# pythoncrazy/jimm

Measured on NVIDIA H100. Metric: images/sec, higher is better.
Workload: dtype f16

## Files before the change

jimm_b200/csrc/common.cuh:

```cuda
#pragma once

#include <cuda.h>
#include <cuda_bf16.h>
#include <cuda_fp16.h>
#include <cuda_fp8.h>
#include <cuda_runtime.h>
#include <stdint.h>

#include <atomic>
#include <mutex>
#include <string>

namespace jimm {

void set_last_error(const char* fmt, ...);

#define JIMM_CUDA_CHECK(expr)                                                                   \
  do {                                                                                          \
    cudaError_t _e = (expr);                                                                    \
    if (_e != cudaSuccess) {                                                                    \
      ::jimm::set_last_error("%s:%d: %s -> %s", __FILE__, __LINE__, #expr, cudaGetErrorString(_e)); \
      return -2;                                                                                \
    }                                                                                           \
  } while (0)
// ... 80 lines not shown
      : "=r"(pred));
  return pred != 0;
}

__device__ __forceinline__ void mbar_init(uint64_t* bar, uint32_t count) {
  asm volatile("mbarrier.init.shared::cta.b64 [%0], %1;" ::"r"(smem_u32(bar)), "r"(count));
}
__device__ __forceinline__ void fence_barrier_init() {
  asm volatile("fence.mbarrier_init.release.cluster;" ::: "memory");
}
__device__ __forceinline__ void fence_proxy_async_smem() {
  asm volatile("fence.proxy.async.shared::cta;" ::: "memory");
}
__device__ __forceinline__ void mbar_arrive(uint64_t* bar) {
  asm volatile("mbarrier.arrive.shared::cta.b64 _, [%0];" ::"r"(smem_u32(bar)) : "memory");
}
__device__ __forceinline__ void mbar_arrive_expect_tx(uint64_t* bar, uint32_t bytes) {
  asm volatile("mbarrier.arrive.expect_tx.shared::cta.b64 _, [%0], %1;" ::"r"(smem_u32(bar)), "r"(bytes) : "memory");
}
__device__ __forceinline__ void mbar_wait(uint64_t* bar, uint32_t parity) {
  asm volatile(
      "{\n\t.reg .pred P1;\n\t"
      "WAIT_LOOP:\n\t"
      "mbarrier.try_wait.parity.shared::cta.b64 P1, [%0], %1;\n\t"
      "@P1 bra DONE;\n\t"
      "bra WAIT_LOOP;\n\t"
      "DONE:\n\t}" ::"r"(smem_u32(bar)),
      "r"(parity)
      : "memory");
}

__device__ __forceinline__ bool mbar_test_wait(uint64_t* bar, uint32_t parity) {
  uint32_t ok;
  asm volatile(
      "{\n\t.reg .pred P1;\n\t"
      "mbarrier.test_wait.parity.shared::cta.b64 P1, [%1], %2;\n\t"
      "selp.u32 %0, 1, 0, P1;\n\t}"
      : "=r"(ok)
      : "r"(smem_u32(bar)), "r"(parity)
      : "memory");
  return ok != 0;
}

__device__ __forceinline__ void tma_prefetch_desc(const CUtensorMap* m) {
  asm volatile("prefetch.tensormap [%0];" ::"l"(reinterpret_cast<uint64_t>(m)) : "memory");
}
__device__ __forceinline__ void tma_load_2d(void* smem_dst, const CUtensorMap* m, uint64_t* bar, int c0, int c1) {
  asm volatile(
      "cp.async.bulk.tensor.2d.shared::cluster.global.mbarrier::complete_tx::bytes [%0], [%1, {%3, %4}], [%2];" ::"r"(
          smem_u32(smem_dst)),
      "l"(reinterpret_cast<uint64_t>(m)), "r"(smem_u32(bar)), "r"(c0), "r"(c1)
      : "memory");
}

__device__ __forceinline__ void tma_store_2d(const CUtensorMap* m, uint32_t smem_src, int c0, int c1) {
  asm volatile("cp.async.bulk.tensor.2d.global.shared::cta.bulk_group [%0, {%2, %3}], [%1];" ::"l"(reinterpret_cast<uint64_t>(m)),
               "r"(smem_src), "r"(c0), "r"(c1)
               : "memory");
}
__device__ __forceinline__ void tma_reduce_add_2d(const CUtensorMap* m, uint32_t smem_src, int c0, int c1) {
  asm volatile("cp.reduce.async.bulk.tensor.2d.global.shared::cta.add.tile.bulk_group [%0, {%2, %3}], [%1];" ::"l"(
                   reinterpret_cast<uint64_t>(m)),
               "r"(smem_src), "r"(c0), "r"(c1)
               : "memory");
}
__device__ __forceinline__ void tma_store_3d(const CUtensorMap* m, uint32_t smem_src, int c0, int c1, int c2) {
  asm volatile("cp.async.bulk.tensor.3d.global.shared::cta.bulk_group [%0, {%2, %3, %4}], [%1];" ::"l"(reinterpret_cast<uint64_t>(m)),
               "r"(smem_src), "r"(c0), "r"(c1), "r"(c2)
               : "memory");
}
__device__ __forceinline__ void tma_reduce_add_3d(const CUtensorMap* m, uint32_t smem_src, int c0, int c1, int c2) {
  asm volatile("cp.reduce.async.bulk.tensor.3d.global.shared::cta.add.tile.bulk_group [%0, {%2, %3, %4}], [%1];" ::"l"(
                   reinterpret_cast<uint64_t>(m)),
               "r"(smem_src), "r"(c0), "r"(c1), "r"(c2)
               : "memory");
}
__device__ __forceinline__ void tma_store_commit() { asm volatile("cp.async.bulk.commit_group;" ::: "memory"); }
__device__ __forceinline__ void tma_store_wait_read() { asm volatile("cp.async.bulk.wait_group.read 0;" ::: "memory"); }
__device__ __forceinline__ void tma_store_wait_read1() { asm volatile("cp.async.bulk.wait_group.read 1;" ::: "memory"); }
__device__ __forceinline__ void tma_store_wait_all() { asm volatile("cp.async.bulk.wait_group 0;" ::: "memory"); }

__device__ __forceinline__ uint32_t cluster_ctarank() {
  uint32_t r;
  asm volatile("mov.u32 %0, %%cluster_ctarank;" : "=r"(r));
  return r;
}
__device__ __forceinline__ void cluster_sync_all() {
  asm volatile("barrier.cluster.arrive.release.aligned;\n\tbarrier.cluster.wait.acquire.aligned;" ::: "memory");
}
__device__ __forceinline__ uint32_t mapa_shared(uint32_t local_smem_addr, uint32_t rank) {
  uint32_t r;
  asm volatile("mapa.shared::cluster.u32 %0, %1, %2;" : "=r"(r) : "r"(local_smem_addr), "r"(rank));
  return r;
}
__device__ __forceinline__ void mbar_arrive_cluster(uint32_t cluster_addr) {
  asm volatile("mbarrier.arrive.release.cluster.shared::cluster.b64 _, [%0];" ::"r"(cluster_addr) : "memory");
}
__device__ __forceinline__ uint64_t make_wgmma_desc_sw128(uint32_t smem_addr) {
  uint64_t d = 0;
  d |= static_cast<uint64_t>((smem_addr & 0x3FFFFu) >> 4);
  d |= static_cast<uint64_t>(1) << 16;
  d |= static_cast<uint64_t>(1024 >> 4) << 32;
  d |= static_cast<uint64_t>(1) << 62;
  return d;
}
template <int SW>
__device__ __forceinline__ uint64_t make_wgmma_desc(uint32_t smem_addr, uint32_t lbo) {
  static_assert(SW == 128 || SW == 64 || SW == 32, "swizzle width");
  constexpr uint64_t layout = SW == 128 ? 1 : SW == 64 ? 2 : 3;
  uint64_t d = 0;
  d |= static_cast<uint64_t>((smem_addr & 0x3FFFFu) >> 4);
  d |= static_cast<uint64_t>((lbo >> 4) & 0x3FFFu) << 16;
  d |= static_cast<uint64_t>(8 * SW >> 4) << 32;
  d |= layout << 62;
  return d;
}
__device__ __forceinline__ void wgmma_fence() { asm volatile("wgmma.fence.sync.aligned;" ::: "memory"); }
__device__ __forceinline__ void wgmma_commit() { asm volatile("wgmma.commit_group.sync.aligned;" ::: "memory"); }
template <int N>
__device__ __forceinline__ void wgmma_wait() { asm volatile("wgmma.wait_group.sync.aligned %0;" ::"n"(N) : "memory"); }
template <int R>
__device__ __forceinline__ void wgmma_fence_operands(float (&d)[R]) {
#pragma unroll
  for (int i = 0; i < R; ++i) asm volatile("" : "+f"(d[i])::"memory");
}

#define JIMM_WGMMA_D128                                                                                                                    \
  "{%0, %1, %2, %3, %4, %5, %6, %7, %8, %9, %10, %11, %12, %13, %14, %15, %16, %17, %18, %19, %20, %21, %22, %23, %24, %25, %26, %27, "     \
  "%28, %29, %30, %31, %32, %33, %34, %35, %36, %37, %38, %39, %40, %41, %42, %43, %44, %45, %46, %47, %48, %49, %50, %51, %52, %53, %54, " \
  "%55, %56, %57, %58, %59, %60, %61, %62, %63, %64, %65, %66, %67, %68, %69, %70, %71, %72, %73, %74, %75, %76, %77, %78, %79, %80, %81, " \
  "%82, %83, %84, %85, %86, %87, %88, %89, %90, %91, %92, %93, %94, %95, %96, %97, %98, %99, %100, %101, %102, %103, %104, %105, %106, "   \
  "%107, %108, %109, %110, %111, %112, %113, %114, %115, %116, %117, %118, %119, %120, %121, %122, %123, %124, %125, %126, %127}"
#define JIMM_WGMMA_D8(i) "+f"(d[i]), "+f"(d[i + 1]), "+f"(d[i + 2]), "+f"(d[i + 3]), "+f"(d[i + 4]), "+f"(d[i + 5]), "+f"(d[i + 6]), "+f"(d[i + 7])
#define JIMM_WGMMA_D128_OPERANDS                                                                                                 \
  JIMM_WGMMA_D8(0), JIMM_WGMMA_D8(8), JIMM_WGMMA_D8(16), JIMM_WGMMA_D8(24), JIMM_WGMMA_D8(32), JIMM_WGMMA_D8(40), JIMM_WGMMA_D8(48), \
      JIMM_WGMMA_D8(56), JIMM_WGMMA_D8(64), JIMM_WGMMA_D8(72), JIMM_WGMMA_D8(80), JIMM_WGMMA_D8(88), JIMM_WGMMA_D8(96),             \
      JIMM_WGMMA_D8(104), JIMM_WGMMA_D8(112), JIMM_WGMMA_D8(120)
template <int KIND>
__device__ __forceinline__ void wgmma_m64n256_ss(float (&d)[128], uint64_t adesc, uint64_t bdesc, uint32_t accumulate) {
  if constexpr (KIND == 0) {
    asm volatile("{\n\t.reg .pred p;\n\tsetp.ne.b32 p, %130, 0;\n\t"
                 "wgmma.mma_async.sync.aligned.m64n256k16.f32.f16.f16 " JIMM_WGMMA_D128 ", %128, %129, p, 1, 1, 0, 0;\n\t}"
                 : JIMM_WGMMA_D128_OPERANDS
                 : "l"(adesc), "l"(bdesc), "r"(accumulate));
  } else if constexpr (KIND == 1) {
    asm volatile("{\n\t.reg .pred p;\n\tsetp.ne.b32 p, %130, 0;\n\t"
                 "wgmma.mma_async.sync.aligned.m64n256k16.f32.bf16.bf16 " JIMM_WGMMA_D128 ", %128, %129, p, 1, 1, 0, 0;\n\t}"
                 : JIMM_WGMMA_D128_OPERANDS
                 : "l"(adesc), "l"(bdesc), "r"(accumulate));
// ... 260 lines not shown
```

jimm_b200/csrc/gemm.cu:

```cuda
#include "gemm.cuh"

#include <stdarg.h>
#include <stdio.h>
#include <stdlib.h>
#include <string.h>

#include <type_traits>

#include "common.cuh"

namespace jimm {

static constexpr int BM = GEMM_TILE_M;
static constexpr int BN = GEMM_TILE_N;
static_assert(BM == 128 && BN == 256, "the warp roles and the wgmma shape below are written for 128 x 256 tiles");
static constexpr int STAGES = 4;
static constexpr int A_STAGE_BYTES = BM * 128;
static constexpr int B_STAGE_BYTES = BN * 128;
static constexpr int STAGE_BYTES = A_STAGE_BYTES + B_STAGE_BYTES;
static constexpr int EPI_WARPS = 8;
static constexpr int EPI_BOX_ROWS = 16;
static constexpr int EPI_BUF_BYTES = EPI_BOX_ROWS * 128;
static constexpr int EPI_BUFS = 2;
static constexpr int EPI_STAGE_BYTES = EPI_WARPS * EPI_BUFS * EPI_BUF_BYTES;
static constexpr int NUM_THREADS = 384;
static constexpr int KERNEL_REGS = 168;

enum OutKind : int { OUT_GENERIC = 0, OUT_H16 = 1, OUT_BF16 = 2, OUT_TF32 = 3, OUT_F32_ADD = 4, OUT_F32 = 5 };

struct EpiDev {
  const float* bias;
  const float* rowadd;
  const float* residual;
  void* out;
  int act, ldr, out_type, ldo, rows_in, rows_out, row_off, mode;
  int M, N;
  int reverse;
  int tok_pad, tok_off;
  const float* ln_scale;
  const float* ln_bias;
  void* ln_out;
  int* ln_cnt;
  int ln_out_type, ln_ldo;
  float ln_eps;
  const float* a_scale;
  const float* b_scale;
};

template <int ACT>
__device__ __forceinline__ float act_ct(float v) {
  if constexpr (ACT == ACT_GELU_TANH) return gelu_tanh(v);
  else if constexpr (ACT == ACT_QUICK_GELU) return quick_gelu(v);
  else return v;
}
__device__ __forceinline__ float apply_act(float v, int act) {
  if (act == ACT_GELU_TANH) return gelu_tanh(v);
  if (act == ACT_QUICK_GELU) return quick_gelu(v);
  return v;
}

__device__ __forceinline__ void remap_row(const EpiDev& e, int row, int& out_row, int& add_row) {
  if (e.rows_in > 0) {
    int b = row / e.rows_in, p = row - b * e.rows_in;
    out_row = b * e.rows_out + p + e.row_off;
    add_row = p + e.row_off;
  } else {
    out_row = row;
    add_row = row;
  }
}

// ... 239 lines not shown
    int out_row, add_row;
    remap_row(epi, row, out_row, add_row);
    float sa = 1.f;
    if constexpr (SCALED) sa = __ldg(epi.a_scale + row);
#pragma unroll
    for (int j = 0; j < NC / 8; ++j) {
#pragma unroll
      for (int q = 0; q < 2; ++q) {
        const int col = n_tile0 + 8 * j + 2 * t + q;
        if (col < epi.N) {
          float v = acc[4 * j + 2 * h + q];
          if constexpr (SCALED) v *= sa * __ldg(epi.b_scale + col);
          if (epi.bias) v += __ldg(epi.bias + col);
          v = apply_act(v, epi.act);
          if (epi.rowadd) v += __ldg(epi.rowadd + static_cast<size_t>(add_row) * epi.N + col);
          if (epi.residual) v += epi.residual[static_cast<size_t>(out_row) * epi.ldr + col];
          store1(epi, out_row, col, v);
        }
      }
    }
  }
}


template <typename T, int OUT, int ACT>
__global__ void __launch_bounds__(NUM_THREADS, 1)
gemm_wgmma_kernel(const __grid_constant__ CUtensorMap map_a, const __grid_constant__ CUtensorMap map_b,
                  const __grid_constant__ CUtensorMap map_c, const EpiDev epi, int K) {
  constexpr bool SCALED = kScaled<T>;
  constexpr int BK = 128 / sizeof(T);
  constexpr int UK = 32 / sizeof(T);
  constexpr int TM = tile_rows(Traits<T>::DTYPE);
  constexpr int STAGE_TX = TM * 128 + B_STAGE_BYTES;
  constexpr int WG_DM = SCALED ? 0 : 64;
  constexpr int WG_DN = SCALED ? 128 : 0;
  constexpr int NC = BN - WG_DN;
  constexpr bool FUSE_LN = OUT == OUT_F32_ADD && ACT == ACT_FUSE_LN;
  constexpr int EPI_ACT = ACT == ACT_FUSE_LN ? static_cast<int>(ACT_NONE) : ACT;
  constexpr int PRODUCER_REGS = FUSE_LN ? 152 : 40;
  constexpr int CONSUMER_REGS = FUSE_LN ? 176 : 232;
  static_assert(128 * PRODUCER_REGS + 256 * CONSUMER_REGS <= NUM_THREADS * KERNEL_REGS, "register split exceeds the CTA's allocation");

  extern __shared__ uint8_t smem_raw[];
  uint8_t* smem = reinterpret_cast<uint8_t*>((reinterpret_cast<uintptr_t>(smem_raw) + 1023) & ~static_cast<uintptr_t>(1023));
  uint8_t* smem_a = smem;
  uint8_t* smem_b = smem + STAGES * A_STAGE_BYTES;
  uint8_t* epi_stage = smem + STAGES * STAGE_BYTES;
  LnQueue* lnq = reinterpret_cast<LnQueue*>(epi_stage + EPI_STAGE_BYTES);
  uint64_t* full_bar = reinterpret_cast<uint64_t*>(lnq + 1);
  uint64_t* empty_bar = full_bar + STAGES;

  const int warp_idx = threadIdx.x >> 5;
  const int lane = threadIdx.x & 31;
  const int M = epi.M, N = epi.N;
  const int m_tiles = (M + TM - 1) / TM, n_tiles = (N + BN - 1) / BN;
  const int num_tiles = m_tiles * n_tiles;
  const int num_kb = (K + BK - 1) / BK;

  pdl_launch_dependents();
  if (warp_idx == 0 && lane == 0) {
    tma_prefetch_desc(&map_a);
    tma_prefetch_desc(&map_b);
    if constexpr (OUT != OUT_GENERIC) tma_prefetch_desc(&map_c);
    for (int s = 0; s < STAGES; ++s) {
      mbar_init(&full_bar[s], 1);
      mbar_init(&empty_bar[s], EPI_WARPS);
    }
    fence_barrier_init();
  }
  if constexpr (FUSE_LN) {
    if (warp_idx == 1) {
      for (int i = lane; i < LNQ; i += 32) lnq->slot[i] = -1;
      if (lane == 0) lnq->head = lnq->tail = lnq->done = 0;
    }
  }
  __syncthreads();
  pdl_wait();

  if (warp_idx < 4) {
    setmaxnreg<KERNEL_REGS, PRODUCER_REGS>();
    if (warp_idx == 0) {
      if (lane == 0) {
        int stage = 0;
        uint32_t phase = 0;
        for (int tile = blockIdx.x; tile < num_tiles; tile += gridDim.x) {
          const int tv = epi.reverse ? num_tiles - 1 - tile : tile;
          const int m_blk = tv / n_tiles, n_blk = tv - m_blk * n_tiles;
          for (int kb = 0; kb < num_kb; ++kb) {
            mbar_wait(&empty_bar[stage], phase ^ 1);
            mbar_arrive_expect_tx(&full_bar[stage], STAGE_TX);
            tma_load_2d(smem_a + stage * A_STAGE_BYTES, &map_a, &full_bar[stage], kb * BK, m_blk * TM);
            tma_load_2d(smem_b + stage * B_STAGE_BYTES, &map_b, &full_bar[stage], kb * BK, n_blk * BN);
            if (++stage == STAGES) { stage = 0; phase ^= 1; }
          }
        }
      }
    } else if constexpr (FUSE_LN) {
      ln_worker<T>(epi, lnq, lane);
    }
  } else {
    setmaxnreg<KERNEL_REGS, CONSUMER_REGS>();
    const int wg = (warp_idx - 4) >> 2;
    const int wq = warp_idx & 3;
    uint8_t* tbuf0 = epi_stage + (warp_idx - 4) * EPI_BUFS * EPI_BUF_BYTES;
    int stage = 0;
    uint32_t phase = 0, box_count = 0;
    int ln_rg = -1, ln_cols = 0;
    float acc[NC / 2];
    for (int tile = blockIdx.x; tile < num_tiles; tile += gridDim.x) {
      const int tv = epi.reverse ? num_tiles - 1 - tile : tile;
      const int m_blk = tv / n_tiles, n_blk = tv - m_blk * n_tiles;
      int prev = -1;
      if constexpr (SCALED) {
#pragma unroll
        for (int i = 0; i < NC / 2; ++i) acc[i] = 0.f;
      }
      for (int kb = 0; kb < num_kb; ++kb) {
        mbar_wait(&full_bar[stage], phase);
        const uint64_t adesc = make_wgmma_desc_sw128(smem_u32(smem_a + stage * A_STAGE_BYTES + wg * WG_DM * 128));
        const uint64_t bdesc = make_wgmma_desc_sw128(smem_u32(smem_b + stage * B_STAGE_BYTES + wg * WG_DN * 128));
        if constexpr (SCALED) {
          float slab[NC / 2];
          wgmma_fence_operands(slab);
          wgmma_fence();
#pragma unroll
          for (int k = 0; k < BK / UK; ++k)
            wgmma_m64n128k32_e4m3_ss(slab, adesc + static_cast<uint64_t>(2 * k), bdesc + static_cast<uint64_t>(2 * k), k != 0 ? 1u : 0u);
          wgmma_commit();
          wgmma_wait<0>();
          wgmma_fence_operands(slab);
          if (lane == 0) mbar_arrive(&empty_bar[stage]);
#pragma unroll
          for (int i = 0; i < NC / 2; ++i) acc[i] += slab[i];
        } else {
          wgmma_fence_operands(acc);
          wgmma_fence();
#pragma unroll
          for (int k = 0; k < BK / UK; ++k)
            wgmma_m64n256_ss<Traits<T>::KIND>(acc, adesc + static_cast<uint64_t>(2 * k), bdesc + static_cast<uint64_t>(2 * k), (kb | k) != 0 ? 1u : 0u);
          wgmma_commit();
          wgmma_fence_operands(acc);
          if (prev >= 0) {
            wgmma_wait<1>();
            if (lane == 0) mbar_arrive(&empty_bar[prev]);
          }
          prev = stage;
        }
        if (++stage == STAGES) { stage = 0; phase ^= 1; }
      }
      if constexpr (!SCALED) {
        wgmma_wait<0>();
        wgmma_fence_operands(acc);
        if (lane == 0) mbar_arrive(&empty_bar[prev]);
      }

      const int row_base = m_blk * TM + wg * WG_DM + wq * 16;
      const int n_tile0 = n_blk * BN + wg * WG_DN;
      if constexpr (OUT == OUT_GENERIC) {
        epilogue_generic<SCALED, NC>(epi, acc, lane, row_base, n_tile0);
      } else {
        if (row_base < M && (WG_DN == 0 || n_tile0 < N))
          epilogue_tma<OUT, EPI_ACT, SCALED, NC>(&map_c, epi, acc, tbuf0, lane, row_base, n_tile0, box_count);
        if constexpr (FUSE_LN) {
          if (lane == 0 && ln_rg >= 0) ln_publish(epi, lnq, ln_rg, ln_cols);
          ln_rg = (row_base & ~31) < M ? row_base >> 5 : -1;
          ln_cols = min(BN, N - n_tile0);
        }
      }
    }
    if constexpr (FUSE_LN) {
      if (lane == 0) {
        if (ln_rg >= 0) ln_publish(epi, lnq, ln_rg, ln_cols);
        __threadfence_block();
        atomicAdd(&lnq->done, 1);
      }
    }
    if constexpr (OUT != OUT_GENERIC) {
      if (lane == 0) tma_store_wait_all();
    }
  }
}

template <typename T>
__global__ void gemm_simt_kernel(const T* __restrict__ A, int lda, const T* __restrict__ B, int ldb, int K, EpiDev epi) {
  __shared__ float As[16][17], Bs[16][17];
  const int tx = threadIdx.x, ty = threadIdx.y;
  const int row = blockIdx.y * 16 + ty, col = blockIdx.x * 16 + tx;
  float acc = 0.f;
  for (int k0 = 0; k0 < K; k0 += 16) {
    const int ar = blockIdx.y * 16 + ty, ak = k0 + tx;
    As[ty][tx] = (ar < epi.M && ak < K) ? to_float(A[static_cast<size_t>(ar) * lda + ak]) : 0.f;
    const int br = blockIdx.x * 16 + ty, bk = k0 + tx;
    Bs[ty][tx] = (br < epi.N && bk < K) ? to_float(B[static_cast<size_t>(br) * ldb + bk]) : 0.f;
    __syncthreads();
#pragma unroll
    for (int k = 0; k < 16; ++k) acc += As[ty][k] * Bs[tx][k];
    __syncthreads();
  }
  if (row < epi.M && col < epi.N) {
    int out_row, add_row;
    remap_row(epi, row, out_row, add_row);
    float v = acc;
    if constexpr (kScaled<T>) v *= epi.a_scale[row] * epi.b_scale[col];
    if (epi.bias) v += epi.bias[col];
    v = apply_act(v, epi.act);
    if (epi.rowadd) v += epi.rowadd[static_cast<size_t>(add_row) * epi.N + col];
    if (epi.residual) v += epi.residual[static_cast<size_t>(out_row) * epi.ldr + col];
    store1(epi, out_row, col, v);
  }
}

static constexpr int SMEM_BYTES = STAGES * STAGE_BYTES + EPI_STAGE_BYTES + static_cast<int>(sizeof(LnQueue)) + 2 * STAGES * 8 + 1024;
static_assert(SMEM_BYTES <= 232448, "exceeds 227 KB of shared memory");
typedef CUresult (*PFN_encodeTiled)(CUtensorMap*, CUtensorMapDataType, cuuint32_t, void*, const cuuint64_t*, const cuuint64_t*,
                                    const cuuint32_t*, const cuuint32_t*, CUtensorMapInterleave, CUtensorMapSwizzle,
                                    CUtensorMapL2promotion, CUtensorMapFloatOOBfill);

static PFN_encodeTiled get_encode_fn() {
  static std::atomic<PFN_encodeTiled> fn{nullptr};
  if (PFN_encodeTiled f = fn.load(std::memory_order_acquire)) return f;
  void* p = nullptr;
  cudaDriverEntryPointQueryResult qres;
  cudaError_t e = cudaGetDriverEntryPoint("cuTensorMapEncodeTiled", &p, cudaEnableDefault, &qres);
  if (e != cudaSuccess || qres != cudaDriverEntryPointSuccess || p == nullptr) {
    set_last_error("cudaGetDriverEntryPoint(cuTensorMapEncodeTiled) failed: %s", cudaGetErrorString(e));
    return nullptr;
  }
  fn.store(reinterpret_cast<PFN_encodeTiled>(p), std::memory_order_release);
  return reinterpret_cast<PFN_encodeTiled>(p);
}

static CUtensorMapDataType tensor_map_dtype(int dtype) {
  switch (dtype) {
// ... 39 lines not shown
  if (r != CUDA_SUCCESS) { set_last_error("cuTensorMapEncodeTiled(3d) failed: CUresult %d", static_cast<int>(r)); return -3; }
  return 0;
}

int device_sm_count() {
  static std::atomic<int> sms[DeviceOnce::kMaxDevices] = {};
  int dev = 0;
  cudaGetDevice(&dev);
  if (dev < 0 || dev >= DeviceOnce::kMaxDevices) dev = 0;
  int n = sms[dev].load(std::memory_order_relaxed);
  if (n == 0) {
    cudaDeviceGetAttribute(&n, cudaDevAttrMultiProcessorCount, dev);
    const char* env = getenv("JIMM_NUM_SMS");
    if (env && atoi(env) > 0) n = atoi(env);
    sms[dev].store(n, std::memory_order_relaxed);
  }
  return n;
}

static int check_epi(const GemmEpilogue& e, int N) {
  if (e.out == nullptr) { set_last_error("gemm: null output"); return -1; }
  if (e.ldo < N) { set_last_error("gemm: ldo (%d) < N (%d)", e.ldo, N); return -1; }
  return 0;
}
static int check_e4m3_epi(const GemmEpilogue& e) {
  if (e.a_scale == nullptr || e.b_scale == nullptr) { set_last_error("gemm: e4m3 operands need row scales for A and B"); return -1; }
  if ((reinterpret_cast<uintptr_t>(e.b_scale) & 7) != 0) { set_last_error("gemm: the B scales must be 8-byte aligned"); return -1; }
  if (e.residual || e.rowadd || e.rows_in != 0 || e.tok_pad != 0 || e.ln_cnt) {
    set_last_error("gemm: e4m3 operands support bias and activation epilogues only (no residual, row-add, row remap, token scatter or "
                   "fused LayerNorm)");
    return -1;
  }
  return 0;
}
int gemm_plan_init(GemmPlan* plan, int dtype, const void* A, int lda, const void* B, int ldb, int M, int N, int K,
                   const GemmEpilogue& epi) {
  if (M <= 0 || N <= 0 || K <= 0) { set_last_error("gemm: bad shape %dx%dx%d", M, N, K); return -1; }
  if (int rc = check_epi(epi, N)) return rc;
  if (dtype == DT_E4M3) {
    if (int rc = check_e4m3_epi(epi)) return rc;
  }
  if (epi.tok_pad != 0) {
    if (epi.tok_pad < 0 || epi.tok_pad % EPI_BOX_ROWS != 0 || M % epi.tok_pad != 0 || epi.tok_off < 0 || epi.tok_S <= 0) {
      set_last_error("gemm: token scatter needs tok_pad a positive multiple of %d dividing M (tok_pad=%d M=%d tok_off=%d tok_S=%d)", EPI_BOX_ROWS,
                     epi.tok_pad, M, epi.tok_off, epi.tok_S);
      return -1;
    }
    if (epi.residual != epi.out || epi.ldr != epi.ldo || epi.out_type != DT_F32) {
      set_last_error("gemm: token scatter reduce-adds into an fp32 output that is also the residual");
      return -1;
    }
  }
  if (int rc = make_tensor_map_2d(&plan->map_a, dtype, A, M, K, lda, tile_rows(dtype))) return rc;
  if (int rc = make_tensor_map_2d(&plan->map_b, dtype, B, N, K, ldb, BN)) return rc;
  plan->M = M; plan->N = N; plan->K = K; plan->dtype = dtype; plan->epi = epi;
  memset(&plan->map_c, 0, sizeof(plan->map_c));
  if (plan->epi.mode == 2) {
    const size_t es = dtype_size(epi.out_type);
    const bool ok = epi.rowadd == nullptr && epi.rows_in == 0 && (static_cast<size_t>(N) * es) % 16 == 0 &&
                    (epi.residual == nullptr || (epi.residual == epi.out && epi.ldr == epi.ldo && epi.out_type == DT_F32)) &&
                    (static_cast<size_t>(epi.ldo) * es) % 16 == 0 && (reinterpret_cast<uintptr_t>(epi.out) & 15) == 0 &&
                    (epi.bias == nullptr || ((reinterpret_cast<uintptr_t>(epi.bias) & 15) == 0 && N % 4 == 0)) &&
                    !(epi.residual && epi.act != ACT_NONE);
    if (ok && epi.tok_pad > 0) {
      if (int rc = make_tensor_map_3d(&plan->map_c, DT_F32, epi.out, M / epi.tok_pad, epi.tok_S, N, epi.ldo)) return rc;
    } else if (ok) {
      if (int rc = make_tensor_map_2d(&plan->map_c, epi.out_type, epi.out, M, N, epi.ldo, EPI_BOX_ROWS)) return rc;
    } else {
      plan->epi.mode = 0;
    }
  }
  if (epi.tok_pad > 0 && plan->epi.mode != 2) {
    set_last_error("gemm: the token scatter needs the TMA epilogue (mode 2, no activation, 16-byte aligned output / bias, N %% 4 == 0)");
    return -1;
  }
  return 0;
}

static EpiDev to_dev(const GemmEpilogue& e, int M, int N) {
  EpiDev d;
  d.bias = e.bias; d.rowadd = e.rowadd; d.residual = e.residual; d.out = e.out;
  d.act = e.act; d.ldr = e.ldr; d.out_type = e.out_type; d.ldo = e.ldo;
  d.rows_in = e.rows_in; d.rows_out = e.rows_out; d.row_off = e.row_off; d.mode = e.mode;
  d.M = M; d.N = N;
  d.tok_pad = e.tok_pad; d.tok_off = e.tok_off;
  d.reverse = e.reverse;
  d.ln_scale = e.ln_scale; d.ln_bias = e.ln_bias; d.ln_out = e.ln_out; d.ln_cnt = e.ln_cnt;
  d.ln_out_type = e.ln_out_type; d.ln_ldo = e.ln_ldo; d.ln_eps = e.ln_eps;
  d.a_scale = e.a_scale; d.b_scale = e.b_scale;
  return d;
}

template <typename T, int OUT, int ACT>
static int launch_one(const GemmPlan* p, int M, cudaStream_t stream) {
  auto* kernel = gemm_wgmma_kernel<T, OUT, ACT>;
  constexpr int TM = tile_rows(Traits<T>::DTYPE);
  static DeviceOnce attr_set;
  if (int rc = attr_set.run([&]() -> int {
        JIMM_CUDA_CHECK(cudaFuncSetAttribute(kernel, cudaFuncAttributeMaxDynamicSharedMemorySize, SMEM_BYTES));
        cudaFuncAttributes fa;
        JIMM_CUDA_CHECK(cudaFuncGetAttributes(&fa, kernel));
        if (fa.numRegs != KERNEL_REGS) {
          set_last_error("gemm: kernel compiled with %d registers per thread, the warpgroup register split assumes %d", fa.numRegs, KERNEL_REGS);
          return -2;
        }
        return 0;
      }))
    return rc;
  const int tiles = ((M + TM - 1) / TM) * ((p->N + BN - 1) / BN);
  const int grid = tiles < device_sm_count() ? tiles : device_sm_count();
  JIMM_CUDA_CHECK(launch_k(kernel, dim3(grid), dim3(NUM_THREADS), SMEM_BYTES, stream, 1, true, p->map_a, p->map_b, p->map_c,
                           to_dev(p->epi, M, p->N), p->K));
  note_launch();
  return 0;
}

template <typename T, int OUT>
static int launch_act(const GemmPlan* p, int M, cudaStream_t stream) {
  switch (p->epi.act) {
    case ACT_GELU_TANH: return launch_one<T, OUT, ACT_GELU_TANH>(p, M, stream);
    case ACT_QUICK_GELU: return launch_one<T, OUT, ACT_QUICK_GELU>(p, M, stream);
    default: return launch_one<T, OUT, ACT_NONE>(p, M, stream);
  }
}

template <typename T>
static int launch_tc(const GemmPlan* p, int M, cudaStream_t stream) {
  const GemmEpilogue& e = p->epi;
  if (e.mode != 2) return launch_one<T, OUT_GENERIC, ACT_NONE>(p, M, stream);
  if constexpr (!kScaled<T>) {
    if (e.residual) return gemm_fuses_ln(p, M) ? launch_one<T, OUT_F32_ADD, ACT_FUSE_LN>(p, M, stream) : launch_one<T, OUT_F32_ADD, ACT_NONE>(p, M, stream);
  }
  switch (e.out_type) {
    case DT_F16: return launch_act<T, OUT_H16>(p, M, stream);
    case DT_BF16: return launch_act<T, OUT_BF16>(p, M, stream);
    case DT_TF32: return launch_act<T, OUT_TF32>(p, M, stream);
    default: return launch_act<T, OUT_F32>(p, M, stream);
  }
}

int gemm_fuses_ln(const GemmPlan* p, int ) {
  const int nv = p->N >> 7;
  const bool width_ok = p->N % 128 == 0 && (nv <= 4 || nv == 6 || nv == 8 || nv == 9);
  const int want = p->dtype == DT_F16 ? DT_F16 : p->dtype == DT_BF16 ? DT_BF16 : DT_TF32;
  return p->epi.ln_cnt != nullptr && p->epi.ln_out_type == want && width_ok && p->epi.mode == 2 && p->epi.residual != nullptr && p->epi.tok_pad == 0;
}

int gemm_plan_run(const GemmPlan* p0, int M_override, cudaStream_t stream, int reverse) {
  const int M = (M_override > 0 && M_override <= p0->M) ? M_override : p0->M;
  if (p0->epi.tok_pad > 0 && M % p0->epi.tok_pad != 0) {
    set_last_error("gemm: token scatter runs whole samples (M=%d, tok_pad=%d)", M, p0->epi.tok_pad);
    return -1;
  }
  GemmPlan local;
  const GemmPlan* p = p0;
  if (reverse != p0->epi.reverse) { local = *p0; local.epi.reverse = reverse; p = &local; }
  switch (p->dtype) {
    case DT_F16: return launch_tc<__half>(p, M, stream);
    case DT_BF16: return launch_tc<__nv_bfloat16>(p, M, stream);
    case DT_F32:
    case DT_TF32: return launch_tc<float>(p, M, stream);
    case DT_E4M3: return launch_tc<__nv_fp8_e4m3>(p, M, stream);
  }
  set_last_error("gemm: bad dtype %d", p->dtype);
// ... 21 lines not shown
```

jimm_b200/csrc/gemm.cuh:

```cuda
#pragma once
#include <cuda.h>
#include <cuda_runtime.h>
#include <stdint.h>

namespace jimm {

enum DType : int { DT_F32 = 0, DT_F16 = 1, DT_BF16 = 2, DT_TF32 = 3, DT_E4M3 = 4 };
enum Act : int { ACT_NONE = 0, ACT_GELU_TANH = 1, ACT_QUICK_GELU = 2 };

inline size_t dtype_size(int dt) { return (dt == DT_F32 || dt == DT_TF32) ? 4 : dt == DT_E4M3 ? 1 : 2; }

constexpr int GEMM_TILE_M = 128;
constexpr int GEMM_TILE_N = 256;

struct GemmEpilogue {
  const float* bias = nullptr;
  int act = ACT_NONE;
  const float* rowadd = nullptr;
  const float* residual = nullptr;
  int ldr = 0;
  void* out = nullptr;
  int out_type = DT_F32;
  int ldo = 0;
  int tok_pad = 0, tok_off = 0, tok_S = 0;
  int reverse = 0;
  int rows_in = 0, rows_out = 0, row_off = 0;
  int mode = 2;
  const float* ln_scale = nullptr;
  const float* ln_bias = nullptr;
  void* ln_out = nullptr;
  int ln_out_type = DT_F16, ln_ldo = 0;
  float ln_eps = 1e-6f;
  int* ln_cnt = nullptr;
  const float* a_scale = nullptr;
  const float* b_scale = nullptr;
};

struct GemmPlan {
  CUtensorMap map_a, map_b, map_c;
  int M = 0, N = 0, K = 0;
  int dtype = DT_F16;
  GemmEpilogue epi;
};

int gemm_plan_init(GemmPlan* plan, int dtype, const void* A, int lda, const void* B, int ldb, int M, int N, int K,
                   const GemmEpilogue& epi);
int gemm_plan_run(const GemmPlan* plan, int M_override, cudaStream_t stream, int reverse = 0);

int gemm_simt_run(int dtype, const void* A, int lda, const void* B, int ldb, int M, int N, int K, const GemmEpilogue& epi,
                  cudaStream_t stream);

int gemm_fuses_ln(const GemmPlan* plan, int M_override);

int device_sm_count();

}
```

jimm_b200/csrc/model.cu:

```cuda
#include <stdarg.h>
#include <stdio.h>
#include <stdlib.h>
#include <string.h>

#include <algorithm>
#include <atomic>
#include <cmath>
#include <map>
#include <tuple>
#include <memory>
#include <utility>
#include <string>
#include <vector>

#include "../../include/jimm_b200.h"
#include "comm.cuh"
#include "common.cuh"
#include "gemm.cuh"
#include "kernels.cuh"

namespace jimm {

static thread_local char g_err[1024] = "";
void set_last_error(const char* fmt, ...) {
// ... 1600 lines not shown
int jimm_encoder_forward(jimm_model_t* m, const float* x, int B, int S, float* out, void* stream) {
  JIMM_TRY(check_sub(m, JIMM_ENCODER, B, S, x, out));
  cudaStream_t s = static_cast<cudaStream_t>(stream);
  const size_t row = static_cast<size_t>(S) * m->vis.D;
  return for_chunks(B, m->max_batch, [&](int b0, int nb) {
    JIMM_CUDA_CHECK(cudaMemcpyAsync(m->ws.enc.x, x + b0 * row, nb * row * sizeof(float), cudaMemcpyDeviceToDevice, s));
    JIMM_TRY(run_encoder(m, &m->vis.enc, nb, S, s, m->ws.enc));
    JIMM_CUDA_CHECK(cudaMemcpyAsync(out + b0 * row, m->ws.enc.x, nb * row * sizeof(float), cudaMemcpyDeviceToDevice, s));
    return 0;
  });
}

int jimm_map_head_forward(jimm_model_t* m, const float* x, int B, int S, float* out, void* stream) {
  JIMM_TRY(check_sub(m, JIMM_MAPHEAD, B, S, x, out));
  cudaStream_t s = static_cast<cudaStream_t>(stream);
  const size_t row = static_cast<size_t>(S) * m->vis.D;
  return for_chunks(B, m->max_batch, [&](int b0, int nb) {
    JIMM_TRY(cast_run(x + b0 * row, m->ws.enc.h, m->cdt, nb * row, s));
    return run_map_head(m, nb, S, out + static_cast<size_t>(b0) * m->vis.D, s);
  });
}

static int ensure_copy_stream(jimm_model* m) {
  if (m->copy_stream) return 0;
  JIMM_CUDA_CHECK(cudaStreamCreateWithFlags(&m->copy_stream, cudaStreamNonBlocking));
  for (int i = 0; i < jimm_model::kHostSlices; ++i) {
    JIMM_CUDA_CHECK(cudaEventCreateWithFlags(&m->ev_copied[i], cudaEventDisableTiming));
    JIMM_CUDA_CHECK(cudaEventCreateWithFlags(&m->ev_consumed[i], cudaEventDisableTiming));
  }
  JIMM_CUDA_CHECK(cudaEventCreateWithFlags(&m->ev_start, cudaEventDisableTiming));
  return 0;
}

static void host_slices(const jimm_model* m, int nb, int* sizes, size_t bytes_per_image = 0) {
  for (int i = 0; i < jimm_model::kHostSlices; ++i) sizes[i] = 0;
  sizes[0] = nb;
  if (const char* env = getenv("JIMM_HOST_SLICES")) {
    int k = 0, acc = 0;
    for (const char* q = env; *q && k < jimm_model::kHostSlices - 1;) {
      const int v = atoi(q);
      if (v <= 0 || acc + v >= nb) break;
      sizes[k++] = v;
      acc += v;
      while (*q && *q != ',') ++q;
      if (*q == ',') ++q;
    }
    sizes[k] = nb - acc;
    return;
  }
  if (nb < 128) return;
  if (bytes_per_image && static_cast<size_t>(nb) * bytes_per_image < (static_cast<size_t>(64) << 20)) return;
  static const int head_div = [] { const char* env = getenv("JIMM_HOST_HEAD_DIV"); return (env && atoi(env) > 0) ? atoi(env) : 4; }();
  const int S = m->vis.S, D = m->vis.D, Mm = m->vis.enc.c.M;
  const int sms = device_sm_count();
  auto cost = [&](int n) {
    const long mt = (static_cast<long>(n) * S + GEMM_TILE_M - 1) / GEMM_TILE_M;
    auto rounds = [&](int N) { return (mt * ((N + GEMM_TILE_N - 1) / GEMM_TILE_N) + sms - 1) / sms; };
    return static_cast<double>(D) * rounds(3 * D) + static_cast<double>(D) * rounds(D) + static_cast<double>(D) * rounds(Mm) +
           static_cast<double>(Mm) * rounds(D);
  };
  int best = nb / head_div;
  double best_cost = 1e30;
  for (int c0 = nb / head_div; c0 <= nb / 3; ++c0) {
    const double cst = cost(c0) + cost(nb - c0) + 1e-3 * c0 * D;
    if (cst < best_cost) { best_cost = cst; best = c0; }
  }
  sizes[0] = best;
  sizes[1] = nb - best;
}

static int vit_forward_host_impl(jimm_model_t* m, const void* img_host, int in_dtype, int B, float* out_host, cudaStream_t s,
                                 jimm_preproc_t* pre, int Hin, int Win) {
  JIMM_TRY(ensure_copy_stream(m));
  const size_t img_elems = static_cast<size_t>(m->vis.img) * m->vis.img * m->vis.C;
  const size_t src_bytes = pre ? static_cast<size_t>(Hin) * Win * 3 : img_elems * dtype_size(in_dtype);
  const int tower_dtype = pre ? (m->cdt == DT_TF32 ? JIMM_F32 : m->cdt) : in_dtype;
  const int od = vision_out_dim(m);
  const int kind = pre ? 1 : 0;
  if (pre) {
    const size_t need = static_cast<size_t>(m->max_batch) * src_bytes;
    if (need > m->ws.in_u8_bytes) {
      std::lock_guard<std::mutex> no_capture(g_capture_mu);
      JIMM_CUDA_CHECK(cudaDeviceSynchronize());
      if (m->ws.in_u8) cudaFree(m->ws.in_u8);
      m->ws.in_u8 = nullptr; m->ws.in_u8_bytes = 0;
      JIMM_CUDA_CHECK(cudaMalloc(&m->ws.in_u8, need));
      m->ws.in_u8_bytes = need;
      m->host_chain = false;
    }
  }
  return for_chunks(B, m->max_batch, [&](int b0, int nb) {
    int sizes[jimm_model::kHostSlices];
    host_slices(m, nb, sizes, src_bytes);
    if (pre && img_elems % 4) {
      for (int i = 0; i + 1 < jimm_model::kHostSlices && sizes[i + 1] > 0; ++i) {
        const int r = sizes[i] % 4;
        sizes[i] -= r;
        sizes[i + 1] += r;
      }
    }
    bool same_layout = m->host_chain && m->host_chain_stream == s && m->host_chain_kind == kind;
    for (int i = 0; i < jimm_model::kHostSlices; ++i) same_layout = same_layout && sizes[i] == m->host_chain_sizes[i];
    if (!same_layout) {
      JIMM_CUDA_CHECK(cudaEventRecord(m->ev_start, s));
      JIMM_CUDA_CHECK(cudaStreamWaitEvent(m->copy_stream, m->ev_start, 0));
      for (int i = 0; i < jimm_model::kHostSlices; ++i) {
        if (m->slot_recorded[i]) JIMM_CUDA_CHECK(cudaStreamWaitEvent(m->copy_stream, m->ev_consumed[i], 0));
        m->slot_recorded[i] = false;
        m->host_chain_sizes[i] = sizes[i];
      }
// ... 156 lines not shown
```

jimm_b200/csrc/probe.cu:

```cuda
#include "../../include/jimm_b200.h"
#include "common.cuh"
#include "gemm.cuh"

namespace jimm {

int make_tensor_map_2d(CUtensorMap* map, int dtype, const void* ptr, int rows, int cols, int ld, int box_rows);

namespace {

constexpr int PB_STAGES = 12;
constexpr int PB_STAGE_BYTES = 128 * 128;

__device__ __forceinline__ void tma_load_2d_multicast(void* smem_dst, const CUtensorMap* m, uint64_t* bar, int c0, int c1, uint16_t mask) {
  asm volatile(
      "cp.async.bulk.tensor.2d.shared::cluster.global.mbarrier::complete_tx::bytes.multicast::cluster [%0], [%1, {%3, %4}], [%2], %5;" ::"r"(
          smem_u32(smem_dst)),
      "l"(reinterpret_cast<uint64_t>(m)), "r"(smem_u32(bar)), "r"(c0), "r"(c1), "h"(mask)
      : "memory");
}

template <int CS>
__global__ void __launch_bounds__(64, 1) l2_probe_kernel(const __grid_constant__ CUtensorMap map_full, const __grid_constant__ CUtensorMap map_part,
                                                         int mode, int iters, int total_rows) {
  extern __shared__ uint8_t smem_raw[];
  uint8_t* smem = reinterpret_cast<uint8_t*>((reinterpret_cast<uintptr_t>(smem_raw) + 1023) & ~static_cast<uintptr_t>(1023));
  uint64_t* full = reinterpret_cast<uint64_t*>(smem + PB_STAGES * PB_STAGE_BYTES);
  uint64_t* empty = full + PB_STAGES;
  const uint32_t rank = CS > 1 ? cluster_ctarank() : 0;
  const int cluster_id = blockIdx.x / CS;
  const bool shared_writes = CS > 1 && mode == 2;
  if (threadIdx.x == 0) {
    for (int i = 0; i < PB_STAGES; ++i) {
      mbar_init(&full[i], 1);
      mbar_init(&empty[i], shared_writes ? CS : 1);
    }
    fence_barrier_init();
  }
  __syncthreads();
  if (CS > 1) cluster_sync_all();
  const int tiles = total_rows / 128;
  if (threadIdx.x == 0) {
    int st = 0;
    uint32_t ph = 0;
    for (int it = 0; it < iters; ++it) {
      const long long tile = mode == 0 ? (static_cast<long long>(blockIdx.x) * iters + it) : (static_cast<long long>(cluster_id) * iters + it);
      const int row = static_cast<int>((tile * 7919) % tiles) * 128;
      mbar_wait(&empty[st], ph ^ 1);
      mbar_arrive_expect_tx(&full[st], PB_STAGE_BYTES);
      if (mode == 2 && CS > 1) {
        constexpr int part = 128 / CS;
        tma_load_2d_multicast(smem + st * PB_STAGE_BYTES + rank * part * 128, &map_part, &full[st], 0, row + rank * part,
                              static_cast<uint16_t>((1u << CS) - 1));
      } else {
        tma_load_2d(smem + st * PB_STAGE_BYTES, &map_full, &full[st], 0, row);
      }
      if (++st == PB_STAGES) { st = 0; ph ^= 1; }
    }
  } else if (threadIdx.x == 32) {
    int st = 0;
    uint32_t ph = 0;
    for (int it = 0; it < iters; ++it) {
      mbar_wait(&full[st], ph);
      if (shared_writes) {
        for (uint32_t r = 0; r < CS; ++r)
          asm volatile("mbarrier.arrive.relaxed.cluster.shared::cluster.b64 _, [%0];" ::"r"(mapa_shared(smem_u32(&empty[st]), r)) : "memory");
      } else {
        mbar_arrive(&empty[st]);
      }
      if (++st == PB_STAGES) { st = 0; ph ^= 1; }
    }
  }
  __syncthreads();
// ... 48 lines not shown
```

Before: 12250.

## Multicast GEMM B tiles across 2-CTA clusters along M

Launches the persistent wgmma GEMM as clusters of two CTAs that work on adjacent M tiles sharing the same N tile. Each CTA loads half of the B tile and multicasts it to both CTAs, which halves B traffic from L2. Consumers release stage buffers on every CTA's empty barrier, and the grid is now sized by the occupancy limit on clusters. The cost is cluster-wide synchronisation and lockstep scheduling. Odd M tile counts leave a CTA loading an out-of-range M tile, and the host cost model is updated to match.

```diff
diff --git a/jimm_b200/csrc/common.cuh b/jimm_b200/csrc/common.cuh
--- a/jimm_b200/csrc/common.cuh
+++ b/jimm_b200/csrc/common.cuh
@@ -156,6 +156,13 @@
       "l"(reinterpret_cast<uint64_t>(m)), "r"(smem_u32(bar)), "r"(c0), "r"(c1)
       : "memory");
 }
+__device__ __forceinline__ void tma_load_2d_multicast(void* smem_dst, const CUtensorMap* m, uint64_t* bar, int c0, int c1, uint16_t mask) {
+  asm volatile(
+      "cp.async.bulk.tensor.2d.shared::cluster.global.mbarrier::complete_tx::bytes.multicast::cluster [%0], [%1, {%3, %4}], [%2], %5;" ::"r"(
+          smem_u32(smem_dst)),
+      "l"(reinterpret_cast<uint64_t>(m)), "r"(smem_u32(bar)), "r"(c0), "r"(c1), "h"(mask)
+      : "memory");
+}
 
 __device__ __forceinline__ void tma_store_2d(const CUtensorMap* m, uint32_t smem_src, int c0, int c1) {
   asm volatile("cp.async.bulk.tensor.2d.global.shared::cta.bulk_group [%0, {%2, %3}], [%1];" ::"l"(reinterpret_cast<uint64_t>(m)),
@@ -198,7 +205,7 @@
   return r;
 }
 __device__ __forceinline__ void mbar_arrive_cluster(uint32_t cluster_addr) {
-  asm volatile("mbarrier.arrive.release.cluster.shared::cluster.b64 _, [%0];" ::"r"(cluster_addr) : "memory");
+  asm volatile("mbarrier.arrive.shared::cluster.b64 _, [%0];" ::"r"(cluster_addr) : "memory");
 }
 __device__ __forceinline__ uint64_t make_wgmma_desc_sw128(uint32_t smem_addr) {
   uint64_t d = 0;
diff --git a/jimm_b200/csrc/gemm.cu b/jimm_b200/csrc/gemm.cu
--- a/jimm_b200/csrc/gemm.cu
+++ b/jimm_b200/csrc/gemm.cu
@@ -5,6 +5,7 @@
 #include <stdlib.h>
 #include <string.h>
 
+#include <algorithm>
 #include <type_traits>
 
 #include "common.cuh"
@@ -13,10 +14,13 @@
 
 static constexpr int BM = GEMM_TILE_M;
 static constexpr int BN = GEMM_TILE_N;
+static constexpr int CM = GEMM_CLUSTER_M;
 static_assert(BM == 128 && BN == 256, "the warp roles and the wgmma shape below are written for 128 x 256 tiles");
 static constexpr int STAGES = 4;
 static constexpr int A_STAGE_BYTES = BM * 128;
 static constexpr int B_STAGE_BYTES = BN * 128;
+static constexpr int B_PART_ROWS = BN / CM;
+static_assert(B_PART_ROWS * 128 % 1024 == 0, "a B part must be whole 8-row swizzle atoms, so the parts land where one box would");
 static constexpr int STAGE_BYTES = A_STAGE_BYTES + B_STAGE_BYTES;
 static constexpr int EPI_WARPS = 8;
 static constexpr int EPI_BOX_ROWS = 16;
@@ -362,10 +366,18 @@
 
   const int warp_idx = threadIdx.x >> 5;
   const int lane = threadIdx.x & 31;
+  const int rank = static_cast<int>(cluster_ctarank());
   const int M = epi.M, N = epi.N;
   const int m_tiles = (M + TM - 1) / TM, n_tiles = (N + BN - 1) / BN;
-  const int num_tiles = m_tiles * n_tiles;
+  const int num_units = (m_tiles + CM - 1) / CM * n_tiles;
+  const int cluster_id = blockIdx.x / CM, num_clusters = gridDim.x / CM;
   const int num_kb = (K + BK - 1) / BK;
+  auto unit_tile = [&](int unit, int& m_blk, int& n_blk) {
+    const int uv = epi.reverse ? num_units - 1 - unit : unit;
+    const int pair = uv / n_tiles;
+    n_blk = uv - pair * n_tiles;
+    m_blk = pair * CM + rank;
+  };
 
   pdl_launch_dependents();
   if (warp_idx == 0 && lane == 0) {
@@ -374,7 +386,7 @@
     if constexpr (OUT != OUT_GENERIC) tma_prefetch_desc(&map_c);
     for (int s = 0; s < STAGES; ++s) {
       mbar_init(&full_bar[s], 1);
-      mbar_init(&empty_bar[s], EPI_WARPS);
+      mbar_init(&empty_bar[s], CM * EPI_WARPS);
     }
     fence_barrier_init();
   }
@@ -384,7 +396,7 @@
       if (lane == 0) lnq->head = lnq->tail = lnq->done = 0;
     }
   }
-  __syncthreads();
+  cluster_sync_all();
   pdl_wait();
 
   if (warp_idx < 4) {
@@ -393,14 +405,15 @@
       if (lane == 0) {
         int stage = 0;
         uint32_t phase = 0;
-        for (int tile = blockIdx.x; tile < num_tiles; tile += gridDim.x) {
-          const int tv = epi.reverse ? num_tiles - 1 - tile : tile;
-          const int m_blk = tv / n_tiles, n_blk = tv - m_blk * n_tiles;
+        for (int unit = cluster_id; unit < num_units; unit += num_clusters) {
+          int m_blk, n_blk;
+          unit_tile(unit, m_blk, n_blk);
           for (int kb = 0; kb < num_kb; ++kb) {
             mbar_wait(&empty_bar[stage], phase ^ 1);
             mbar_arrive_expect_tx(&full_bar[stage], STAGE_TX);
             tma_load_2d(smem_a + stage * A_STAGE_BYTES, &map_a, &full_bar[stage], kb * BK, m_blk * TM);
-            tma_load_2d(smem_b + stage * B_STAGE_BYTES, &map_b, &full_bar[stage], kb * BK, n_blk * BN);
+            tma_load_2d_multicast(smem_b + stage * B_STAGE_BYTES + rank * B_PART_ROWS * 128, &map_b, &full_bar[stage], kb * BK,
+                                  n_blk * BN + rank * B_PART_ROWS, static_cast<uint16_t>((1u << CM) - 1));
             if (++stage == STAGES) { stage = 0; phase ^= 1; }
           }
         }
@@ -413,13 +426,17 @@
     const int wg = (warp_idx - 4) >> 2;
     const int wq = warp_idx & 3;
     uint8_t* tbuf0 = epi_stage + (warp_idx - 4) * EPI_BUFS * EPI_BUF_BYTES;
+    auto release = [&](int s) {
+#pragma unroll
+      for (int r = 0; r < CM; ++r) mbar_arrive_cluster(mapa_shared(smem_u32(&empty_bar[s]), static_cast<uint32_t>(r)));
+    };
     int stage = 0;
     uint32_t phase = 0, box_count = 0;
     int ln_rg = -1, ln_cols = 0;
     float acc[NC / 2];
-    for (int tile = blockIdx.x; tile < num_tiles; tile += gridDim.x) {
-      const int tv = epi.reverse ? num_tiles - 1 - tile : tile;
-      const int m_blk = tv / n_tiles, n_blk = tv - m_blk * n_tiles;
+    for (int unit = cluster_id; unit < num_units; unit += num_clusters) {
+      int m_blk, n_blk;
+      unit_tile(unit, m_blk, n_blk);
       int prev = -1;
       if constexpr (SCALED) {
 #pragma unroll
@@ -439,7 +456,7 @@
           wgmma_commit();
           wgmma_wait<0>();
           wgmma_fence_operands(slab);
-          if (lane == 0) mbar_arrive(&empty_bar[stage]);
+          if (lane == 0) release(stage);
 #pragma unroll
           for (int i = 0; i < NC / 2; ++i) acc[i] += slab[i];
         } else {
@@ -452,7 +469,7 @@
           wgmma_fence_operands(acc);
           if (prev >= 0) {
             wgmma_wait<1>();
-            if (lane == 0) mbar_arrive(&empty_bar[prev]);
+            if (lane == 0) release(prev);
           }
           prev = stage;
         }
@@ -461,7 +478,7 @@
       if constexpr (!SCALED) {
         wgmma_wait<0>();
         wgmma_fence_operands(acc);
-        if (lane == 0) mbar_arrive(&empty_bar[prev]);
+        if (lane == 0) release(prev);
       }
 
       const int row_base = m_blk * TM + wg * WG_DM + wq * 16;
@@ -489,6 +506,8 @@
       if (lane == 0) tma_store_wait_all();
     }
   }
+  __syncwarp();
+  cluster_sync_all();
 }
 
 template <typename T>
@@ -634,7 +653,7 @@
     }
   }
   if (int rc = make_tensor_map_2d(&plan->map_a, dtype, A, M, K, lda, tile_rows(dtype))) return rc;
-  if (int rc = make_tensor_map_2d(&plan->map_b, dtype, B, N, K, ldb, BN)) return rc;
+  if (int rc = make_tensor_map_2d(&plan->map_b, dtype, B, N, K, ldb, B_PART_ROWS)) return rc;
   plan->M = M; plan->N = N; plan->K = K; plan->dtype = dtype; plan->epi = epi;
   memset(&plan->map_c, 0, sizeof(plan->map_c));
   if (plan->epi.mode == 2) {
@@ -678,6 +697,10 @@
   auto* kernel = gemm_wgmma_kernel<T, OUT, ACT>;
   constexpr int TM = tile_rows(Traits<T>::DTYPE);
   static DeviceOnce attr_set;
+  static int max_clusters[DeviceOnce::kMaxDevices];
+  int dev = 0;
+  cudaGetDevice(&dev);
+  if (dev < 0 || dev >= DeviceOnce::kMaxDevices) dev = 0;
   if (int rc = attr_set.run([&]() -> int {
         JIMM_CUDA_CHECK(cudaFuncSetAttribute(kernel, cudaFuncAttributeMaxDynamicSharedMemorySize, SMEM_BYTES));
         cudaFuncAttributes fa;
@@ -686,12 +709,28 @@
           set_last_error("gemm: kernel compiled with %d registers per thread, the warpgroup register split assumes %d", fa.numRegs, KERNEL_REGS);
           return -2;
         }
+        cudaLaunchConfig_t cfg = {};
+        cudaLaunchAttribute attr;
+        attr.id = cudaLaunchAttributeClusterDimension;
+        attr.val.clusterDim.x = CM;
+        attr.val.clusterDim.y = 1;
+        attr.val.clusterDim.z = 1;
+        cfg.gridDim = dim3(CM);
+        cfg.blockDim = dim3(NUM_THREADS);
+        cfg.dynamicSmemBytes = SMEM_BYTES;
+        cfg.attrs = &attr;
+        cfg.numAttrs = 1;
+        JIMM_CUDA_CHECK(cudaOccupancyMaxActiveClusters(&max_clusters[dev], kernel, &cfg));
+        if (max_clusters[dev] < 1) {
+          set_last_error("gemm: no cluster of %d CTAs of the GEMM kernel fits on device %d", CM, dev);
+          return -2;
+        }
         return 0;
       }))
     return rc;
-  const int tiles = ((M + TM - 1) / TM) * ((p->N + BN - 1) / BN);
-  const int grid = tiles < device_sm_count() ? tiles : device_sm_count();
-  JIMM_CUDA_CHECK(launch_k(kernel, dim3(grid), dim3(NUM_THREADS), SMEM_BYTES, stream, 1, true, p->map_a, p->map_b, p->map_c,
+  const int units = ((M + TM - 1) / TM + CM - 1) / CM * ((p->N + BN - 1) / BN);
+  const int clusters = std::min(std::min(units, max_clusters[dev]), std::max(1, device_sm_count() / CM));
+  JIMM_CUDA_CHECK(launch_k(kernel, dim3(CM * clusters), dim3(NUM_THREADS), SMEM_BYTES, stream, CM, true, p->map_a, p->map_b, p->map_c,
                            to_dev(p->epi, M, p->N), p->K));
   note_launch();
   return 0;
diff --git a/jimm_b200/csrc/gemm.cuh b/jimm_b200/csrc/gemm.cuh
--- a/jimm_b200/csrc/gemm.cuh
+++ b/jimm_b200/csrc/gemm.cuh
@@ -12,6 +12,7 @@
 
 constexpr int GEMM_TILE_M = 128;
 constexpr int GEMM_TILE_N = 256;
+constexpr int GEMM_CLUSTER_M = 2;
 
 struct GemmEpilogue {
   const float* bias = nullptr;
diff --git a/jimm_b200/csrc/model.cu b/jimm_b200/csrc/model.cu
--- a/jimm_b200/csrc/model.cu
+++ b/jimm_b200/csrc/model.cu
@@ -1676,10 +1676,11 @@
   if (bytes_per_image && static_cast<size_t>(nb) * bytes_per_image < (static_cast<size_t>(64) << 20)) return;
   static const int head_div = [] { const char* env = getenv("JIMM_HOST_HEAD_DIV"); return (env && atoi(env) > 0) ? atoi(env) : 4; }();
   const int S = m->vis.S, D = m->vis.D, Mm = m->vis.enc.c.M;
-  const int sms = device_sm_count();
+  const int clusters = device_sm_count() / GEMM_CLUSTER_M;
   auto cost = [&](int n) {
     const long mt = (static_cast<long>(n) * S + GEMM_TILE_M - 1) / GEMM_TILE_M;
-    auto rounds = [&](int N) { return (mt * ((N + GEMM_TILE_N - 1) / GEMM_TILE_N) + sms - 1) / sms; };
+    const long groups = (mt + GEMM_CLUSTER_M - 1) / GEMM_CLUSTER_M;
+    auto rounds = [&](int N) { return (groups * ((N + GEMM_TILE_N - 1) / GEMM_TILE_N) + clusters - 1) / clusters; };
     return static_cast<double>(D) * rounds(3 * D) + static_cast<double>(D) * rounds(D) + static_cast<double>(D) * rounds(Mm) +
            static_cast<double>(Mm) * rounds(D);
   };
diff --git a/jimm_b200/csrc/probe.cu b/jimm_b200/csrc/probe.cu
--- a/jimm_b200/csrc/probe.cu
+++ b/jimm_b200/csrc/probe.cu
@@ -10,14 +10,6 @@
 
 constexpr int PB_STAGES = 12;
 constexpr int PB_STAGE_BYTES = 128 * 128;
-
-__device__ __forceinline__ void tma_load_2d_multicast(void* smem_dst, const CUtensorMap* m, uint64_t* bar, int c0, int c1, uint16_t mask) {
-  asm volatile(
-      "cp.async.bulk.tensor.2d.shared::cluster.global.mbarrier::complete_tx::bytes.multicast::cluster [%0], [%1, {%3, %4}], [%2], %5;" ::"r"(
-          smem_u32(smem_dst)),
-      "l"(reinterpret_cast<uint64_t>(m)), "r"(smem_u32(bar)), "r"(c0), "r"(c1), "h"(mask)
-      : "memory");
-}
 
 template <int CS>
 __global__ void __launch_bounds__(64, 1) l2_probe_kernel(const __grid_constant__ CUtensorMap map_full, const __grid_constant__ CUtensorMap map_part,
```

Measured after the change: 12190 (median of 6 runs). No clear change (-0.4%).
